# sjpollard/video-how-do-your-tokens-merge

Measured on AMD Instinct MI355X. Metric: clips/sec at r=16, VideoMAE-B 16x224x224 (forward with ToMe merge; merge indices bit-exact against the fp32-arithmetic oracle, which the reference's fp32 fixtures pin), higher is better.
Workload: dtype bf16; 1 GPU; VideoMAE-B random-init, synthetic 16x224x224 clips, r=16, bf16 (BASELINE.json configs[1]); r=16, parallelism=dp1: independent replicas, one RCCL all-reduce of [top1, top5, clips], step_launch=eager

## Files before the change

include/tome_hip.h:

```cpp
#ifndef TOME_HIP_H
#define TOME_HIP_H

#include <stddef.h>
#include <stdint.h>

#ifdef __cplusplus
extern "C" {
#endif

typedef void *tome_stream_t;

enum tome_dtype { TOME_F32 = 0, TOME_BF16 = 1, TOME_F16 = 2 };

enum tome_mode { TOME_SUM = 0, TOME_MEAN = 1, TOME_AMAX = 2, TOME_PROD = 3, TOME_AMIN = 4 };

enum tome_status {
    TOME_OK = 0,
    TOME_EINVAL = 1,
    TOME_EWORKSPACE = 2,
    TOME_ELAUNCH = 3
};

#define TOME_ABI_VERSION 11

// ... 105 lines not shown
                                  const int32_t *row_map, int drop, void *grad_in, tome_stream_t stream);

size_t tome_layernorm_backward_workspace_bytes(int64_t rows, int64_t C);
int tome_layernorm_backward(const void *gy, const void *xs, const void *gx_in, int dtype, int64_t groups,
                            int64_t group_rows, int skip_first, int64_t C, const void *weight, float eps, void *gx,
                            void *dweight, void *dbias, void *workspace, tome_stream_t stream);

size_t tome_layernorm_backward_regrouped_workspace_bytes(int64_t B, int64_t F, int64_t P, int64_t C);
int tome_layernorm_backward_regrouped(const void *gy, const void *xs, const void *gx_in, int dtype, int64_t B, int64_t F,
                                      int64_t P, int64_t C, const void *weight, float eps, void *gx, void *dweight,
                                      void *dbias, void *workspace, tome_stream_t stream);

int tome_add_layernorm_amp(const void *x, int x_dtype, const void *addend, int addend_dtype, int64_t groups,
                           int64_t group_rows, int skip_first, int64_t C, const void *weight_f32, const void *bias_f32,
                           float eps, void *x_out, void *y_out, int y_dtype, tome_stream_t stream);

size_t tome_layernorm_backward_amp_workspace_bytes(int64_t rows, int64_t C, int x_dtype);
int tome_layernorm_backward_amp(const void *gy, int gy_dtype, const void *xs, const void *gx_in, int x_dtype,
                                int64_t groups, int64_t group_rows, int skip_first, int64_t C, const void *weight_f32,
                                float eps, void *gx, void *gx16, void *dweight_f32, void *dbias_f32, void *workspace,
                                tome_stream_t stream);

size_t tome_prop_attention_backward_workspace_bytes(int64_t B, int64_t H, int64_t N, int64_t Nk);
int tome_prop_attention_backward(const void *q, const void *k, const void *v, const void *out, const void *dout,
                                 int dtype, int64_t B, int64_t H, int64_t N, int64_t Nk, int64_t D,
                                 const int64_t *q_strides, const int64_t *k_strides, const int64_t *v_strides,
                                 const int64_t *out_strides, const int64_t *dout_strides, const float *log_size,
                                 int64_t log_size_stride, int bias_skip, float scale, void *dq, void *dk, void *dv,
                                 const int64_t *dq_strides, const int64_t *dk_strides, const int64_t *dv_strides,
                                 void *workspace, size_t workspace_bytes, tome_stream_t stream);

size_t tome_prop_attention_segments_backward_workspace_bytes(int64_t B, int64_t H, int64_t N, int64_t Nk, int64_t nseg);
int tome_prop_attention_segments_backward(const void *q, const void *k, const void *v, const void *out, const void *dout,
                                          int dtype, int64_t B, int64_t H, int64_t N, int64_t Nk, int64_t D,
                                          const int64_t *q_strides, const int64_t *k_strides, const int64_t *v_strides,
                                          const int64_t *out_strides, const int64_t *dout_strides, const float *log_size,
                                          int64_t log_size_stride, float scale, int64_t nseg, const int64_t *seg_strides,
                                          const int64_t *grad_seg_strides, void *dq, void *dk, void *dv,
                                          const int64_t *dq_strides, const int64_t *dk_strides, const int64_t *dv_strides,
                                          void *workspace, size_t workspace_bytes, tome_stream_t stream);

int tome_trajectory_mix_backward(const void *q2, const void *k2, const void *val, const void *dout, int dtype, int64_t B,
                                 int64_t S, int64_t F, int64_t H, int64_t D, int64_t k_row_stride, int64_t v_row_stride,
                                 int64_t dout_batch_stride, float scale, void *dq2, void *dk2, void *dval,
                                 int64_t dk_row_stride, int64_t dv_row_stride, tome_stream_t stream);

int tome_short_attention_backward(const void *q, const void *k, const void *v, const void *dout, int dtype, int64_t B,
                                  int64_t H, int64_t N, int64_t D, const int64_t *q_strides, const int64_t *k_strides,
                                  const int64_t *v_strides, float scale, void *dq, void *dk, void *dv,
                                  const int64_t *dq_strides, const int64_t *dk_strides, const int64_t *dv_strides,
                                  tome_stream_t stream);

int tome_gelu_erf(const void *x, int dtype, int64_t elements, void *y, tome_stream_t stream);

size_t tome_gelu_erf_backward_workspace_bytes(int64_t rows, int64_t width);
int tome_gelu_erf_backward(const void *h, const void *ga, int dtype, int64_t rows, int64_t width, void *gh, void *act,
                           void *dbias, void *workspace, size_t workspace_bytes, tome_stream_t stream);

int tome_gelu_tanh(const void *x, int dtype, int64_t elements, void *y, tome_stream_t stream);
int tome_gelu_tanh_backward(const void *h, const void *ga, int dtype, int64_t rows, int64_t width, void *gh, void *act,
                            void *dbias, void *workspace, size_t workspace_bytes, tome_stream_t stream);

int tome_tubelet_rows(const void *x, int elem_bytes, int64_t B, int64_t C, int64_t T, int64_t H, int64_t W,
                      const int64_t *x_strides, int64_t kt, int64_t kh, int64_t kw, void *rows,
                      tome_stream_t stream);

int tome_row_map(int64_t n, int64_t T, int64_t r, int distill_token, const int64_t *src_idx,
                 const int64_t *dst_idx, const int64_t *unm_idx, int32_t *row_map, tome_stream_t stream);
int tome_source_init(int64_t n, int64_t T, int64_t r, int distill_token, int drop, const int32_t *row_map,
                     float *source_out, tome_stream_t stream);

size_t tome_partition_workspace_bytes(int64_t n, int64_t Na, int64_t Nb, int64_t D);
int tome_match_partition(const void *metric, int dtype, int64_t n, int64_t T, int64_t D, int64_t stride_n,
                         int64_t stride_t, int64_t k, const int64_t *a_idx, const int64_t *b_idx, int64_t Na,
                         int64_t Nb, int64_t *dst_idx, int32_t *offsets, int32_t *sources, void *workspace,
                         size_t workspace_bytes, tome_stream_t stream);
int tome_merge_partition(const void *x, int dtype, int64_t n, int64_t T, int64_t C, int64_t k, const int64_t *a_idx,
                         const int64_t *b_idx, int64_t Na, int64_t Nb, const int32_t *offsets,
                         const int32_t *sources, int mode, void *out, tome_stream_t stream);
int tome_merge_wavg_partition(const void *x, int x_dtype, const void *size, int size_dtype, int64_t n, int64_t T,
                              int64_t C, int64_t k, const int64_t *a_idx, const int64_t *b_idx, int64_t Na,
                              int64_t Nb, const int32_t *offsets, const int32_t *sources, void *x_out,
                              void *size_out, void *log_size_out, tome_stream_t stream);
int tome_unmerge_partition(const void *x, int dtype, int64_t n, int64_t T, int64_t C, int64_t k,
                           const int64_t *a_idx, const int64_t *b_idx, int64_t Na, int64_t Nb,
                           const int64_t *dst_idx, void *out, tome_stream_t stream);

#ifdef TOME_PROFILE_HOOKS
int tome_profile_enable(int on);
int tome_profile_read(float *stage_ms, int max_stages);
#endif

#ifdef __cplusplus
}
#endif
#endif
```

video-how-do-your-tokens-merge_amd/csrc/tome_kernels.hip:

```cpp
#include <hip/hip_runtime.h>
#include <stdarg.h>
#include <stdint.h>
#include <stdio.h>
#include <stdlib.h>
#include <string.h>

#include <type_traits>

#include "../../include/tome_hip.h"
#include "tome_common.h"
#include "tome_match.h"
#include "tome_match_filter.h"
#include "tome_merge.h"
#include "tome_merge_bwd.h"
#include "tome_ln_bwd.h"
#include "tome_gelu_bwd.h"
#include "tome_partition.h"
#include "tome_attn.h"
#include "tome_attn_stream.h"
#include "tome_attn_resident.h"
#include "tome_attn_bwd.h"
#include "tome_short_attn_bwd.h"
#include "tome_traj_bwd.h"
#include "tome_embed.h"

static thread_local char g_err[512] = "";

static int fail(int code, const char *fmt, ...) {
    va_list ap;
    va_start(ap, fmt);
    vsnprintf(g_err, sizeof(g_err), fmt, ap);
    va_end(ap);
    return code;
}

static int check_launch(const char *what) {
    hipError_t e = hipGetLastError();
    if (e != hipSuccess) return fail(TOME_ELAUNCH, "%s: %s", what, hipGetErrorString(e));
    return TOME_OK;
}

extern "C" int tome_abi_version(void) { return TOME_ABI_VERSION; }
extern "C" const char *tome_last_error(void) { return g_err; }

extern "C" int64_t tome_effective_r(int64_t T, int64_t r, int class_token, int distill_token) {
    int64_t prot = (class_token ? 1 : 0) + (distill_token ? 1 : 0);
    int64_t avail = T - prot;
    int64_t cap = avail >= 0 ? avail / 2 : -((-avail + 1) / 2);
    int64_t re = r < cap ? r : cap;
    return re < 0 ? 0 : re;
}

static inline size_t align_up(size_t v, size_t a) { return (v + a - 1) / a * a; }
static inline bool aligned16(const void *p) { return ((uintptr_t)p & 15) == 0; }

template <typename T> struct Dt { using type = T; };
template <int V> using Op = std::integral_constant<int, V>;

template <bool F32, typename F, typename Bad>
static int dispatch_x(int dtype, F &&f, Bad &&bad) {
    switch (dtype) {
    case TOME_F32:
        if constexpr (F32) return f(Dt<float>{});
        break;
    case TOME_BF16: return f(Dt<bf16_t>{});
    case TOME_F16: return f(Dt<f16_t>{});
    }
    return bad();
}
// ... 1260 lines not shown
        return fail(TOME_EINVAL, "tome_short_attention_backward: bad shape/pointer");
    if (D != 64 || N > SHORT_MAXN)
        return fail(TOME_EINVAL, "tome_short_attention_backward: head dim 64 and at most %d tokens per sequence",
                    SHORT_MAXN);
    if (int rc = not_16bit("tome_short_attention_backward", dtype, "tensors")) return rc;
    const int64_t *strides[6] = {q_strides, k_strides, v_strides, dq_strides, dk_strides, dv_strides};
    const void *ptrs[7] = {q, k, v, dout, dq, dk, dv};
    if (int rc = check_short_rows("tome_short_attention_backward", strides, 6, ptrs, 7)) return rc;
    for (int i = 3; i < 6; ++i)
        if ((B > 1 && strides[i][0] < H * 64) || (N > 1 && strides[i][2] < H * 64))
            return fail(TOME_EINVAL, "tome_short_attention_backward: rows of dq / dk / dv overlap");
    const int64_t units = B * H;
    const int64_t blocks = (units + 31) / 32;
    if (blocks > 0x7fffffffLL) return fail(TOME_EINVAL, "tome_short_attention_backward: too many sequences");
    const ShortBwdStrides s{q_strides[0],  q_strides[2],  k_strides[0],  k_strides[2],  v_strides[0],  v_strides[2],
                            dq_strides[0], dq_strides[2], dk_strides[0], dk_strides[2], dv_strides[0], dv_strides[2]};
    hipStream_t st = (hipStream_t)stream;
    return dispatch_x<false>(dtype, [&](auto tx) {
        using TX = typename decltype(tx)::type;
        hipLaunchKernelGGL(k_short_attention_bwd<TX>, dim3((unsigned)blocks), dim3(256), 0, st, (const TX *)q,
                           (const TX *)k, (const TX *)v, (const TX *)dout, s, units, (int)H, (int)N, scale, (TX *)dq,
                           (TX *)dk, (TX *)dv);
        return check_launch("k_short_attention_bwd");
    }, [&] { return not_16bit("tome_short_attention_backward", dtype, "tensors"); });
}

template <int FORM>
static int gelu_impl(const char *who, const void *x, int dtype, int64_t elements, void *y, tome_stream_t stream) {
    if (!x || !y || elements <= 0) return fail(TOME_EINVAL, "%s: bad shape/pointer", who);
    if (int rc = not_16bit(who, dtype, "tensors")) return rc;
    if (elements % 8 || !aligned16(x) || !aligned16(y))
        return fail(TOME_EINVAL, "%s: a multiple of 8 elements in 16-byte aligned buffers required", who);
    const int64_t chunks = elements / 8;
    const int64_t blocks = (chunks + 1023) / 1024;
    if (blocks > 0x7fffffffLL) return fail(TOME_EINVAL, "%s: too large", who);
    hipStream_t st = (hipStream_t)stream;
    return dispatch_x<false>(dtype, [&](auto tx) {
        using TX = typename decltype(tx)::type;
        if (FORM == GELU_TANH) {
            hipLaunchKernelGGL(k_gelu_tanh<TX>, dim3((unsigned)blocks), dim3(256), 0, st, (const TX *)x, (TX *)y, chunks);
            return check_launch("k_gelu_tanh");
        }
        hipLaunchKernelGGL(k_gelu_erf<TX>, dim3((unsigned)blocks), dim3(256), 0, st, (const TX *)x, (TX *)y, chunks);
        return check_launch("k_gelu_erf");
    }, [&] { return not_16bit(who, dtype, "tensors"); });
}

extern "C" int tome_gelu_erf(const void *x, int dtype, int64_t elements, void *y, tome_stream_t stream) {
    return gelu_impl<GELU_ERF>("tome_gelu_erf", x, dtype, elements, y, stream);
}

extern "C" int tome_gelu_tanh(const void *x, int dtype, int64_t elements, void *y, tome_stream_t stream) {
    return gelu_impl<GELU_TANH>("tome_gelu_tanh", x, dtype, elements, y, stream);
}

#define GELU_BWD_MAX_PARTS 512
#define GELU_BWD_MAX_WIDTH 8192
struct GeluBwdForm { int S; int U; int RP; int64_t spw; int64_t parts; };
static GeluBwdForm gelu_bwd_form(int64_t rows, int64_t width) {
    const int64_t cpr = width / 8;
    const int S = (int)((cpr + 255) / 256);
    const int U = S == 1 ? 4 : (S <= 3 ? 2 : 1);
    const int RP = S == 1 ? (int)(256 / cpr) : 1;
    const int64_t passes = (rows + RP - 1) / RP;
    const int64_t steps = (passes + U - 1) / U;
    const int64_t spw = (steps + GELU_BWD_MAX_PARTS - 1) / GELU_BWD_MAX_PARTS;
    return GeluBwdForm{S, U, RP, spw, (steps + spw - 1) / spw};
}

static bool gelu_bwd_shape_ok(int64_t rows, int64_t width) {
    return rows >= 1 && rows <= 0x7fffffffLL && width >= 8 && width % 8 == 0 && width <= GELU_BWD_MAX_WIDTH;
}

extern "C" size_t tome_gelu_erf_backward_workspace_bytes(int64_t rows, int64_t width) {
    if (!gelu_bwd_shape_ok(rows, width)) return 0;
    return align_up((size_t)gelu_bwd_form(rows, width).parts * (size_t)width * sizeof(float), 256);
}

template <int FORM>
static int gelu_backward_impl(const char *who, const void *h, const void *ga, int dtype, int64_t rows, int64_t width,
                              void *gh, void *act, void *dbias, void *workspace, size_t workspace_bytes,
                              tome_stream_t stream) {
    if (!h || !ga || !gh) return fail(TOME_EINVAL, "%s: null buffer", who);
    if (int rc = not_16bit(who, dtype, "tensors")) return rc;
    if (!gelu_bwd_shape_ok(rows, width))
        return fail(TOME_EINVAL, "%s: width %% 8 == 0, width <= 8192 and 1 .. 2^31 - 1 rows required", who);
    if (!aligned16(h) || !aligned16(ga) || !aligned16(gh) || !aligned16(act) || !aligned16(dbias) ||
        !aligned16(workspace))
        return fail(TOME_EINVAL, "%s: 16-byte aligned buffers required", who);
    if (act && (act == h || act == ga || act == gh))
        return fail(TOME_EINVAL, "%s: the activation needs a buffer of its own", who);
    if (gh == h) return fail(TOME_EINVAL, "%s: gh may lie over ga, not over h", who);
    if (dbias && (!workspace || workspace_bytes < tome_gelu_erf_backward_workspace_bytes(rows, width)))
        return fail(TOME_EWORKSPACE, "%s: the bias gradient needs a workspace of "
                                     "tome_gelu_erf_backward_workspace_bytes()", who);
    const int64_t cpr = width / 8, chunks = rows * cpr;
    hipStream_t st = (hipStream_t)stream;
    return dispatch_x<false>(dtype, [&](auto tx) {
        using TX = typename decltype(tx)::type;
        auto with_act = [&](auto launch) { return act ? launch(Op<1>{}) : launch(Op<0>{}); };
        if (!dbias) {
            const int64_t blocks = (chunks + 1023) / 1024;
            return with_act([&](auto a) {
                hipLaunchKernelGGL((k_gelu_bwd<TX, 1, false, decltype(a)::value != 0, FORM>), dim3((unsigned)blocks),
                                   dim3(256), 0, st, (const TX *)h, (const TX *)ga, chunks, 256, 1, 1, (TX *)gh, (TX *)act,
                                   (float *)nullptr);
// ... 343 lines not shown
```

video-how-do-your-tokens-merge_amd/tome/_abi.py:

```python
from __future__ import annotations

import ctypes
import os
from typing import Optional

import torch

_PKG = os.path.dirname(os.path.dirname(os.path.abspath(__file__)))
LIB_PATH = os.environ.get("TOME_HIP_LIB", os.path.join(_PKG, "lib", "libtome_hip.so"))

i64, i32, vp, sz, f32 = ctypes.c_int64, ctypes.c_int, ctypes.c_void_p, ctypes.c_size_t, ctypes.c_float
SIGNATURES = {
    "tome_abi_version": (i32, [], False),
    "tome_last_error": (ctypes.c_char_p, [], False),
    "tome_effective_r": (i64, [i64, i64, i32, i32], False),
    "tome_match_workspace_bytes": (sz, [i64, i64, i64], False),
    "tome_match": (i32, [vp, i32, i64, i64, i64, i64, i64, i64, i32, i32, vp, vp, vp, vp, vp, vp, sz, vp], False),
    "tome_match_keys": (i32, [vp, i32, i64, i64, i64, i64, i64, i64, i64, i64, i64, i64, i32, i32, vp, vp, vp, vp, vp,
                             vp, sz, vp], False),
    "tome_match_scores": (i32, [vp, i64, i64, i64, i32, i32, vp, vp, vp, vp, vp, vp, sz, vp], False),
    "tome_edge_keep": (i32, [vp, vp, i64, i64, i64, f32, vp, vp], False),
    "tome_merge_wavg": (i32, [vp, i32, vp, i32, i64, i64, i64, i64, vp, vp, vp, i32, vp, vp, vp, vp, vp], False),
    "tome_merge_wavg_ln": (i32, [vp, i32, vp, i32, i64, i64, i64, i64, vp, vp, vp, i32, vp, vp, vp, f32, vp, vp, vp, vp,
                                vp, vp, vp], False),
# ... 1 lines not shown
                                       False),
    "tome_merge_wavg_regrouped_ln": (i32, [vp, i32, vp, i32, i64, i64, i64, i64, i64, i32, vp, vp, vp, vp, vp, vp, f32,
                                          vp, i32, vp, vp, vp, vp, vp, vp, vp], False),
    "tome_add_layernorm": (i32, [vp, vp, i32, i64, i64, vp, vp, f32, vp, vp, vp], False),
    "tome_add_layernorm_skip_first": (i32, [vp, vp, i32, i64, i64, i64, vp, vp, f32, vp, vp, vp], False),
    "tome_add_layernorm_regrouped": (i32, [vp, vp, i32, i64, i64, i64, i64, vp, vp, f32, vp, vp, vp], False),
    "tome_prop_attention": (i32, [vp, vp, vp, i32, i64, i64, i64, i64, i64, vp, vp, vp, vp, i64, i32, f32, vp, vp, vp],
                                 False),
    "tome_prop_attention_segments": (i32, [vp, vp, vp, i32, i64, i64, i64, i64, i64, vp, vp, vp, vp, i64, f32, vp, vp,
                                          i64, vp, vp], False),
    "tome_trajectory_mix": (i32, [vp, vp, vp, i32, i64, i64, i64, i64, i64, i64, i64, f32, vp, i64, vp, vp], False),
    "tome_short_attention": (i32, [vp, vp, vp, i32, i64, i64, i64, i64, vp, vp, vp, f32, vp, vp], False),
    "tome_merge": (i32, [vp, i32, i64, i64, i64, i64, vp, vp, vp, i32, i32, vp, vp, vp], False),
    "tome_drop": (i32, [vp, i32, i64, i64, i64, i64, vp, i32, vp, vp], False),
    "tome_drop_regrouped": (i32, [vp, i32, i64, i64, i64, i64, i64, i32, vp, vp, vp], False),
    "tome_unmerge": (i32, [vp, i32, i64, i64, i64, i64, vp, vp, vp, vp, vp], False),
    "tome_merge_backward": (i32, [vp, i32, vp, vp, i32, i64, i64, i64, i64, vp, i32, i32, vp, vp], False),
    "tome_merge_backward_regrouped": (i32, [vp, i32, vp, vp, i32, i64, i64, i64, i64, i64, i32, vp, i32, vp, vp],
                                           False),
    "tome_row_map": (i32, [i64, i64, i64, i32, vp, vp, vp, vp, vp], False),
    "tome_source_init": (i32, [i64, i64, i64, i32, i32, vp, vp, vp], False),
    "tome_gelu_erf": (i32, [vp, i32, i64, vp, vp], False),
    "tome_tubelet_rows": (i32, [vp, i32, i64, i64, i64, i64, i64, vp, i64, i64, i64, vp, vp], False),
    "tome_partition_workspace_bytes": (sz, [i64, i64, i64, i64], False),
    "tome_match_partition": (i32, [vp, i32, i64, i64, i64, i64, i64, i64, vp, vp, i64, i64, vp, vp, vp, vp, sz, vp],
                                  False),
    "tome_merge_partition": (i32, [vp, i32, i64, i64, i64, i64, vp, vp, i64, i64, vp, vp, i32, vp, vp], False),
    "tome_merge_wavg_partition": (i32, [vp, i32, vp, i32, i64, i64, i64, i64, vp, vp, i64, i64, vp, vp, vp, vp, vp, vp],
                                       False),
    "tome_unmerge_partition": (i32, [vp, i32, i64, i64, i64, i64, vp, vp, i64, i64, vp, vp, vp], False),
    "tome_layernorm_backward_workspace_bytes": (sz, [i64, i64], True),
    "tome_layernorm_backward": (i32, [vp, vp, vp, i32, i64, i64, i32, i64, vp, f32, vp, vp, vp, vp, vp], True),
    "tome_prop_attention_backward_workspace_bytes": (sz, [i64, i64, i64, i64], True),
    "tome_prop_attention_backward": (i32, [vp, vp, vp, vp, vp, i32, i64, i64, i64, i64, i64, vp, vp, vp, vp, vp, vp,
                                          i64, i32, f32, vp, vp, vp, vp, vp, vp, vp, sz, vp], True),
    "tome_gelu_erf_backward_workspace_bytes": (sz, [i64, i64], True),
    "tome_gelu_erf_backward": (i32, [vp, vp, i32, i64, i64, vp, vp, vp, vp, sz, vp], True),
    "tome_short_attention_backward": (i32, [vp, vp, vp, vp, i32, i64, i64, i64, i64, vp, vp, vp, f32, vp, vp, vp, vp,
                                           vp, vp, vp], True),
    "tome_layernorm_backward_regrouped_workspace_bytes": (sz, [i64, i64, i64, i64], True),
    "tome_layernorm_backward_regrouped": (i32, [vp, vp, vp, i32, i64, i64, i64, i64, vp, f32, vp, vp, vp, vp, vp],
                                               True),
    "tome_prop_attention_segments_backward_workspace_bytes": (sz, [i64, i64, i64, i64, i64], True),
    "tome_prop_attention_segments_backward": (i32, [vp, vp, vp, vp, vp, i32, i64, i64, i64, i64, i64, vp, vp, vp, vp, vp,
                                                   vp, i64, f32, i64, vp, vp, vp, vp, vp, vp, vp, vp, vp, sz, vp], True),
    "tome_trajectory_mix_backward": (i32, [vp, vp, vp, vp, i32, i64, i64, i64, i64, i64, i64, i64, i64, f32, vp, vp, vp,
                                          i64, i64, vp], True),
    "tome_gelu_tanh": (i32, [vp, i32, i64, vp, vp], True),
    "tome_gelu_tanh_backward": (i32, [vp, vp, i32, i64, i64, vp, vp, vp, vp, sz, vp], True),
    "tome_add_layernorm_amp": (i32, [vp, i32, vp, i32, i64, i64, i32, i64, vp, vp, f32, vp, vp, i32, vp], True),
    "tome_layernorm_backward_amp_workspace_bytes": (sz, [i64, i64, i32], True),
    "tome_layernorm_backward_amp": (i32, [vp, i32, vp, vp, i32, i64, i64, i32, i64, vp, f32, vp, vp, vp, vp, vp, vp],
                                         True),
}
SYMBOLS = tuple(SIGNATURES)

ABI_VERSION = 11
DTYPES = {torch.float32: 0, torch.bfloat16: 1, torch.float16: 2}
MODES = {"sum": 0, "mean": 1, "amax": 2, "max": 2, "prod": 3, "amin": 4, "min": 4}

_lib = None


class TomeHipError(RuntimeError):
    pass


def lib() -> ctypes.CDLL:
    global _lib
    if _lib is not None:
        return _lib
    _lib = bind(LIB_PATH)
    return _lib


def bind(path: str) -> ctypes.CDLL:
    if not os.path.exists(path):
        raise TomeHipError(
            f"HIP extension not found at {path}: the MI355X merge path has no fallback. "
            "Build it with `python video-how-do-your-tokens-merge_amd/csrc/build.py` (needs hipcc).")
    L = ctypes.CDLL(path)
    for name, (restype, argtypes, later) in SIGNATURES.items():
        if later and not _exports(L, name):
            continue
        fn = getattr(L, name)
        fn.restype, fn.argtypes = restype, argtypes
    if L.tome_abi_version() != ABI_VERSION:
        raise TomeHipError(f"{os.path.basename(path)} ABI {L.tome_abi_version()} != expected {ABI_VERSION}")
    return L


def _exports(L, name: str) -> bool:
    try:
        getattr(L, name)
    except AttributeError:
        return False
    return True


def require_symbol(L, name: str):
    if not _exports(L, name):
        raise TomeHipError(f"{name} is missing from the loaded library: it reports ABI {ABI_VERSION} but was built before "
                           "this entry was added; rebuild it with `python video-how-do-your-tokens-merge_amd/csrc/build.py`")
    return getattr(L, name)


# ... 824 lines not shown
        rc = entry(q2.data_ptr(), k2.data_ptr(), val.data_ptr(), dout.data_ptr(), dtype_code(q2, "q2"), B, S, F, heads, 64,
                   k2.stride(2), val.stride(2), dout.stride(0) if B > 1 else 0, float(scale), dq2.data_ptr(), _ptr(dk2),
                   _ptr(dval), 0 if dk2 is None else dk2.stride(2), 0 if dval is None else dval.stride(2),
                   _stream(q2.device))
    _check(rc, "tome_trajectory_mix_backward")
    return dq2, dk2, dval


def drop_regrouped(plan: MatchPlan, x_full: torch.Tensor, frames: int, has_cls: bool = True) -> torch.Tensor:
    x_full, B, C, cls, F, P = _prep_regrouped("drop_regrouped", plan, x_full, frames, has_cls)
    out = torch.empty((B, cls + (P - plan.r) * F, C), dtype=x_full.dtype, device=x_full.device)
    with _on_device(x_full.device):
        rc = lib().tome_drop_regrouped(x_full.data_ptr(), dtype_code(x_full, "x"), B, F, P, C, plan.r, cls,
                                       plan.unm_idx.data_ptr(), out.data_ptr(), _stream(x_full.device))
    _check(rc, "tome_drop_regrouped")
    return out


def unmerge(plan: MatchPlan, x: torch.Tensor) -> torch.Tensor:
    x = _prep_x(plan, x, "unmerge(x)", plan.T - plan.r)
    n, _, C = x.shape
    out = torch.empty((n, plan.T, C), dtype=x.dtype, device=x.device)
    with _on_device(x.device):
        rc = lib().tome_unmerge(x.data_ptr(), dtype_code(x, "x"), n, plan.T, C, plan.r, plan.src_idx.data_ptr(),
                                plan.dst_idx.data_ptr(), plan.unm_idx.data_ptr(), out.data_ptr(), _stream(x.device))
    _check(rc, "tome_unmerge")
    return out


def gelu_ok(x: torch.Tensor) -> bool:
    return (x.is_cuda and x.dtype in (torch.bfloat16, torch.float16) and x.is_contiguous() and x.numel() % 8 == 0
            and x.numel() > 0 and x.data_ptr() % 16 == 0 and not (torch.is_grad_enabled() and needs_grad(x)))


def _gelu(name: str, x: torch.Tensor, inplace: bool) -> torch.Tensor:
    if not gelu_ok(x):
        raise TomeHipError(f"{name}: contiguous 16-bit device tensor with a multiple of 8 elements required")
    entry = require_symbol(lib(), "tome_" + name)
    y = x if inplace else torch.empty_like(x)
    with _on_device(x.device):
        rc = entry(x.data_ptr(), dtype_code(x, "x"), x.numel(), y.data_ptr(), _stream(x.device))
    _check(rc, "tome_" + name)
    return y


def gelu_erf(x: torch.Tensor, inplace: bool = False) -> torch.Tensor:
    return _gelu("gelu_erf", x, inplace)


def gelu_tanh(x: torch.Tensor, inplace: bool = False) -> torch.Tensor:
    return _gelu("gelu_tanh", x, inplace)


GELU_BWD_MAX_WIDTH = 8192


def mlp_trainable(y: torch.Tensor, fc1, fc2, act) -> bool:
    from ._mlp import _stock_module
    if not (_stock_module(fc1, torch.nn.Linear) and _stock_module(fc2, torch.nn.Linear)
            and _stock_module(act, torch.nn.GELU) and getattr(act, "approximate", "none") == "none"):
        return False
    return mlp_tensors_trainable(y, fc1, fc2)


def mlp_tensors_trainable(y: torch.Tensor, fc1, fc2) -> bool:
    C, Hd = fc1.in_features, fc1.out_features
    params = [fc1.weight, fc2.weight] + [b for b in (fc1.bias, fc2.bias) if b is not None]
    return (y.is_cuda and y.dtype in (torch.bfloat16, torch.float16) and y.dim() >= 2 and y.shape[-1] == C
            and y.numel() > 0 and fc2.in_features == Hd and Hd % 8 == 0 and Hd <= GELU_BWD_MAX_WIDTH
            and (C * y.element_size()) % 16 == 0 and (fc2.out_features * y.element_size()) % 16 == 0
            and all(p.dtype == y.dtype and p.device == y.device for p in params))


def _gelu_backward(name: str, h: torch.Tensor, ga: torch.Tensor, want_act: bool, want_bias: bool, inplace: bool):
    require_device(h, f"{name}(h)")
    if h.dtype not in (torch.bfloat16, torch.float16):
        raise TomeHipError(f"{name}: 16-bit tensors only, got {h.dtype}")
    Hd = h.shape[-1] if h.dim() >= 2 else 0
    if Hd == 0 or Hd % 8 or Hd > GELU_BWD_MAX_WIDTH or h.numel() == 0:
        raise TomeHipError(f"{name}: h must be [..., Hd] with Hd % 8 == 0 and Hd <= {GELU_BWD_MAX_WIDTH}, "
                           f"got {tuple(h.shape)}")
    if ga.shape != h.shape or ga.dtype != h.dtype or ga.device != h.device:
        raise TomeHipError(f"{name}: ga must have h's shape, dtype and device")
    if not h.is_contiguous() or not ga.is_contiguous():
        raise TomeHipError(f"{name}: contiguous tensors required")
    h, ga = h.detach(), ga.detach()
    rows = h.numel() // Hd
    L = lib()
    entry = require_symbol(L, "tome_" + name)
    gh = ga if inplace else torch.empty_like(ga)
    act = torch.empty_like(h) if want_act else None
    dbias = torch.empty(Hd, dtype=h.dtype, device=h.device) if want_bias else None
    with _on_device(h.device):
        stream = _stream(h.device)
        ws = _sized_workspace(L, "tome_gelu_erf_backward_workspace_bytes", (rows, Hd), h.device, stream,
                              name) if want_bias else None
        rc = entry(h.data_ptr(), ga.data_ptr(), dtype_code(h, "h"), rows, Hd, gh.data_ptr(), _ptr(act), _ptr(dbias),
                   _ptr(ws), 0 if ws is None else ws.numel(), stream)
    _check(rc, "tome_" + name)
    return gh, act, dbias


def gelu_erf_backward(h: torch.Tensor, ga: torch.Tensor, *, want_act: bool, want_bias: bool, inplace: bool = True):
    return _gelu_backward("gelu_erf_backward", h, ga, want_act, want_bias, inplace)


# ... 328 lines not shown
```

video-how-do-your-tokens-merge_amd/tome/patch/_common.py:

```python
from __future__ import annotations

import os
import threading
from typing import Callable, Dict, Tuple

import torch

from .. import _abi, _attn, _ln, _mlp, _overlap
from .._mlp import _plain_mlp, _stock_module
from ..merge import (bipartite_soft_matching, bipartite_soft_matching_drop, bipartite_soft_matching_hybrid,
                     drop_regrouped, merge_source, merge_wavg, merge_wavg_regrouped)
from ..utils import parse_r

_SUBCLASSES: Dict[Tuple[type, str], type] = {}
_FUSE_LN = os.environ.get("TOME_FUSE_LN", "1") != "0"
_FUSE_ADD = os.environ.get("TOME_FUSE_ADD", "1") != "0"
_FUSE_NEXT = os.environ.get("TOME_FUSE_NEXT", "1") != "0"
_ATTN_KERNEL = os.environ.get("TOME_ATTN_KERNEL", "1") != "0"
_GELU_KERNEL = os.environ.get("TOME_GELU_KERNEL", "1") != "0"
_FUSE_FC2 = os.environ.get("TOME_FUSE_FC2", "1") != "0"
_SKIP_FIRST = os.environ.get("TOME_SKIP_FIRST", "1") != "0"


def swizzle(module: torch.nn.Module, tag: str, methods: dict) -> None:
    base = module.__class__
    if getattr(base, "_tome_tag", None) == tag:
        return
    key = (base, tag)
    sub = _SUBCLASSES.get(key)
    if sub is None:
        sub = type(tag, (base,), dict(methods, _tome_tag=tag))
        _SUBCLASSES[key] = sub
    module.__class__ = sub


def has_tag(module, tag: str) -> bool:
    return getattr(module.__class__, "_tome_tag", None) == tag


def new_tome_info(trace_source, prop_attn, mode, head_aggregation, threshold, verbose, class_token) -> dict:
    return {
        "r": 0,
        "size": None,
        "source": None,
        "trace_source": trace_source,
        "prop_attn": prop_attn,
        "verbose": verbose,
        "class_token": class_token,
        "distill_token": False,
        "mode": mode,
        "head_aggregation": head_aggregation,
        "threshold": threshold,
    }


_in_flight = {}
_issue_locks: Dict[int, "threading.RLock"] = {}
_issue_locks_guard = threading.Lock()
_warned_two_streams = False


def _current_stream(device):
    cur = torch.cuda.current_stream(device)
    return cur.cuda_stream, cur


def _record_event(stream):
    ev = torch.cuda.Event()
    ev.record(stream)
    return ev


def _guarded(device) -> bool:
# ... 7 lines not shown
            lock = _issue_locks[device.index] = threading.RLock()
        return lock


def _guard_one_forward_in_flight(device) -> None:
    global _warned_two_streams
    sid, cur = _current_stream(device)
    last = _in_flight.get(device.index)
    if last is None or last[0] == sid or last[1].query():
        return
    msg = ("a forward issued on another HIP stream of this process is still in flight: the library GEMMs of two "
           "concurrent forwards never finish on this platform")
    if os.environ.get("TOME_ONE_FORWARD", "order") == "raise":
        raise RuntimeError(msg + ".  Run one forward at a time per process (one process per GPU).")
    cur.wait_event(last[1])
    if not _warned_two_streams:
        _warned_two_streams = True
        import warnings
        warnings.warn(msg + "; this forward has been ordered behind it (no overlap between the two streams).",
                      RuntimeWarning, stacklevel=3)


def _note_forward_issued(device) -> None:
    sid, cur = _current_stream(device)
    _in_flight[device.index] = (sid, _record_event(cur))


class one_forward_at_a_time:

    def __init__(self, device):
        self.device = device
        self.on = device is not None and _guarded(device)

    def __enter__(self):
        if self.on:
            self.lock = _issue_lock(self.device)
            self.lock.acquire()
            try:
                _guard_one_forward_in_flight(self.device)
            except BaseException:
                self.lock.release()
                raise
        return self

    def __exit__(self, *exc):
        if self.on:
            try:
                _note_forward_issued(self.device)
            finally:
                self.lock.release()
        return False


def wrap_model_forward(model_wrapper: torch.nn.Module, blocks_of: Callable) -> None:
    base = model_wrapper.__class__
    if getattr(base, "_tome_tag", None) == "ToMeVisionTransformer":
        return

    def forward(self, *args, **kwdargs):
        param = next(self.parameters(), None)
        with one_forward_at_a_time(None if param is None else param.device):
            self._tome_info["r"] = parse_r(len(blocks_of(self)), self.r)
            self._tome_info["size"] = None
            self._tome_info["source"] = None
            self._tome_info.pop("_prenorm", None)
            self._tome_info.pop("_folded", None)
            try:
                return super(sub, self).forward(*args, **kwdargs)
            finally:
                if param is not None:
                    _overlap.join(param.device)

    sub = type("ToMeVisionTransformer", (base,), {"forward": forward, "_tome_tag": "ToMeVisionTransformer"})
    model_wrapper.__class__ = sub


keys_ready = _overlap.keys_ready
match_beside = _overlap.match_beside


def attention_qkv(qkv, size, scale: float, dropout_p: float = 0.0, bias_skip: bool = False):
    return attention(qkv[0], qkv[1], qkv[2], size, scale, dropout_p, bias_skip, qkv)


def attention(q, k, v, size, scale: float, dropout_p: float = 0.0, bias_skip: bool = False, qkv=None):
    out = _attn.attention(q, k, v, size, scale, dropout_p, bias_skip, qkv) if _ATTN_KERNEL else None
    if out is not None:
        return out
    B, H, N, hd = q.shape
    bias = None
    if size is not None:
        log = _abi.log_of_size(size)[:, None, None, :, 0].to(q.dtype)
        if bias_skip:
            bias = torch.zeros(B, 1, N, N, dtype=q.dtype, device=q.device)
            bias[:, :, 1:, 1:] = log
        else:
            bias = log
    out = torch.nn.functional.scaled_dot_product_attention(q, k, v, attn_mask=bias, dropout_p=dropout_p, scale=scale)
    return out.transpose(1, 2).reshape(B, N, H * hd)


def _mlp_steps(mlp, y):
    return mlp.fc2(_mlp.hidden(mlp, y, _GELU_KERNEL)) if _plain_mlp(mlp) else mlp(y)


def run_mlp(mlp, y):
    out = _mlp.mlp(mlp, y) if _GELU_KERNEL else None
    return _mlp_steps(mlp, y) if out is None else out


def foldable(linear, eval_mode: bool = True):
    if (_FUSE_FC2 and _FUSE_NEXT and eval_mode and _stock_module(linear, torch.nn.Linear) and linear.bias is not None
            and not (torch.is_grad_enabled() and _abi.needs_grad(linear.weight, linear.bias))):
        return linear
    return None


def mlp_residual(block, mlp, x, y, info, scale=None, drop_path=None):
    folded = info.get("_folded")
    waiting = folded is not None and folded[0] is x
    out = _mlp.mlp(mlp, y) if _GELU_KERNEL and not waiting else None
    if out is None:
        if _plain_mlp(mlp) and scale is None and (drop_path is None or not block.training):
            return finish_linear(block, x, _mlp.hidden(mlp, y, _GELU_KERNEL), mlp.fc2, info)
        if waiting:
            raise RuntimeError("the residual stream carries a folded bias, but the block's MLP is not the one it was folded for")
        out = _mlp_steps(mlp, y)
    if scale is not None:
        out = scale * out
    return finish_block(block, x, out if drop_path is None else drop_path(out), info)


def pick_reduction(mode: str, merge_fn, drop_fn, hybrid_fn):
    if mode in ("merge", "random_merge"):
        return merge_fn
    if mode in ("drop", "random_drop"):
        return drop_fn
    if mode in ("hybrid",):
        return hybrid_fn
    raise ValueError(f"unknown ToMe mode {mode!r}")


def reduce_merge(metric, x, info, r):
    merge, _ = bipartite_soft_matching(metric, r, info["class_token"], info["distill_token"], info["mode"])
    if info["trace_source"]:
        info["source"] = merge_source(merge, x, info["source"])
    before = x.size(1)
    x, info["size"] = merge_wavg(merge, x, info["size"], log_size=info["prop_attn"])
    if info["verbose"]:
        print(f"Merged {before} to {x.size(1)} tokens")
    return x


def link_next_norms(blocks, norm_attr: str, tag: str = "ToMeBlock", skip_first: bool = False) -> None:
    blocks = list(blocks)
    for cur, nxt in zip(blocks, blocks[1:]):
        target = getattr(nxt, norm_attr, None) if has_tag(nxt, tag) and nxt is not cur else None
        object.__setattr__(cur, "_tome_next_norm", target)
        object.__setattr__(cur, "_tome_next_skip_first", bool(skip_first) and _SKIP_FIRST)
    if blocks:
        object.__setattr__(blocks[-1], "_tome_next_norm", None)


def first_norm(block, x, info, norm, skip_first: bool = False):
    pre = info.pop("_prenorm", None)
    if pre is not None and pre[0] is x and pre[2] is norm:
        if bool(pre[3]) == bool(skip_first):
            return pre[1]
        if skip_first:
            return pre[1][:, 1:, :]
    out = _ln.add_layernorm(x, None, norm, skip_first) if _FUSE_NEXT else None
    if out is None:
        return norm(x)[:, 1:, :] if skip_first else norm(x)
    _, y, skipped = out
    return y[:, 1:, :] if (skip_first and not skipped) else y


def _hand_over(block, x, addend, info):
    nxt = getattr(block, "_tome_next_norm", None)
    out = None if nxt is None else _ln.add_layernorm(x, addend, nxt, getattr(block, "_tome_next_skip_first", False))
    if out is None:
        return None
    x, h, skipped = out
# ... 215 lines not shown
```

video-how-do-your-tokens-merge_amd/tome/patch/videomae.py:

```python
from __future__ import annotations

import copy

import torch
import torch.nn.functional as F

from . import _common as C
from ..merge import HeadMeanKeys


def _block_forward(self, x):
    info = self._tome_info
    attn_size = info["size"] if info["prop_attn"] else None
    attn, metric = self.attn(C.first_norm(self, x, info, self.norm1), attn_size, info["head_aggregation"])
    if self.gamma_1 is not None:
        attn = self.gamma_1 * attn
    fold = C.foldable(self.mlp.fc2, not self.training) if (self.gamma_2 is None and C._plain_mlp(self.mlp)) else None
    x, y = C.merge_then_norm(metric, x, info, self.norm2, self.reduction_function, videomae_merge,
                             residual=self.drop_path(attn), fold=fold)
    return C.mlp_residual(self, self.mlp, x, y, info, scale=self.gamma_2, drop_path=self.drop_path)


def _duplicate_block_forward(self, x):
    info = self._tome_info
    attn_size = info["size"] if info["prop_attn"] else None
    _, metric = self.attn(self.norm1(x), attn_size, info["head_aggregation"])
    return self.reduction_function(metric, x, info)


def _attention_forward(self, x, size: torch.Tensor = None, head_aggregation: str = "mean"):
    B, N, _ = x.shape
    bias = None
    if self.q_bias is not None:
        bias = torch.cat((self.q_bias, torch.zeros_like(self.v_bias, requires_grad=False), self.v_bias))
    qkv = F.linear(x, self.qkv.weight, bias).reshape(B, N, 3, self.num_heads, -1).permute(2, 0, 3, 1, 4)
    q, k, v = qkv[0], qkv[1], qkv[2]
    drop_p = self.attn_drop.p if self.training else 0.0
    info = getattr(self, "_tome_info", None)
    ready = C.keys_ready(k, info) if head_aggregation == "mean" else None
    out = C.attention_qkv(qkv, size, self.scale, drop_p)
    if head_aggregation == "mean":
        metric = HeadMeanKeys(k)
        C.match_beside(metric, ready, info)
    elif head_aggregation == "concat":
        metric = k.transpose(1, 2).reshape(B, N, -1)
    else:
        raise ValueError(f"head_aggregation {head_aggregation!r}")
    return self.proj_drop(self.proj(out)), metric


def videomae_merge(metric, x, _tome_info):
    r = _tome_info["r"].pop(0)
    return C.reduce_merge(metric, x, _tome_info, r) if r > 0 else x


def videomae_drop(metric, x, _tome_info):
    r = _tome_info["r"].pop(0)
    return C.reduce_drop(metric, x, _tome_info, r) if r > 0 else x


def videomae_hybrid(metric, x, _tome_info):
    r = _tome_info["r"].pop(0)
    return C.reduce_hybrid(metric, x, _tome_info, r) if r > 0 else x


def _is_block(m) -> bool:
    return all(hasattr(m, a) for a in ("attn", "mlp", "norm1", "norm2", "gamma_1"))


def _is_attention(m) -> bool:
    return all(hasattr(m, a) for a in ("qkv", "proj", "num_heads", "q_bias"))


def apply_duplicate_patch(model, layer_to_duplicate, quantity):
    for i in range(layer_to_duplicate, layer_to_duplicate + quantity - 1):
        model.model.blocks.insert(index=i, module=copy.deepcopy(model.model.blocks[i]))
        C.swizzle(model.model.blocks[i], "ToMeDuplicateBlock", {"forward": _duplicate_block_forward})


def apply_patch(model_wrapper, trace_source: bool = False, prop_attn: bool = False, mode: str = "merge",
                head_aggregation: str = "mean", threshold: float = 0.0, verbose: bool = False):
    model = model_wrapper.model
    C.wrap_model_forward(model_wrapper, lambda w: w.model.blocks)
    model_wrapper.r = 0
    model_wrapper._tome_info = C.new_tome_info(trace_source, prop_attn, mode, head_aggregation, threshold, verbose,
                                               class_token=False)
    reduction_function = C.pick_reduction(mode, videomae_merge, videomae_drop, videomae_hybrid)
    for module in model.modules():
        if C.has_tag(module, "ToMeDuplicateBlock"):
            module._tome_info = model_wrapper._tome_info
            module.reduction_function = reduction_function
        elif _is_block(module):
            C.swizzle(module, "ToMeBlock", {"forward": _block_forward})
            module._tome_info = model_wrapper._tome_info
            module.reduction_function = reduction_function
        elif _is_attention(module):
            C.swizzle(module, "ToMeAttention", {"forward": _attention_forward})
            module._tome_info = model_wrapper._tome_info
    C.link_next_norms(model.blocks, "norm1")
```

Measured before the change: 2575 clips/s.

## Pool the last block's MLP output before fc2 using linearity of mean pooling

For the final transformer block in eval mode, the model ends with an identity norm followed by mean pooling and fc_norm. The MLP's fc2 and the residual add are both linear, so the change averages GELU(fc1(y)) and x over tokens with a new HIP token_mean kernel, then runs fc2 once per clip on the pooled vector instead of per token. This drops the per-token fc2 GEMM and the residual write in the last block, and returns a single pooled token so the host's mean step becomes trivial. In exchange it relies on a number of module-type and hook checks, and its rounding differs from the original per-token bf16 path because the sum is accumulated in fp32.

```diff
diff --git a/include/tome_hip.h b/include/tome_hip.h
--- a/include/tome_hip.h
+++ b/include/tome_hip.h
@@ -181,6 +181,9 @@
                                   tome_stream_t stream);
 
 int tome_gelu_erf(const void *x, int dtype, int64_t elements, void *y, tome_stream_t stream);
+
+int tome_token_mean(const void *x, int dtype, int64_t groups, int64_t tokens, int64_t width, int act, float *out,
+                    tome_stream_t stream);
 
 size_t tome_gelu_erf_backward_workspace_bytes(int64_t rows, int64_t width);
 int tome_gelu_erf_backward(const void *h, const void *ga, int dtype, int64_t rows, int64_t width, void *gh, void *act,
diff --git a/video-how-do-your-tokens-merge_amd/csrc/tome_kernels.hip b/video-how-do-your-tokens-merge_amd/csrc/tome_kernels.hip
--- a/video-how-do-your-tokens-merge_amd/csrc/tome_kernels.hip
+++ b/video-how-do-your-tokens-merge_amd/csrc/tome_kernels.hip
@@ -15,6 +15,7 @@
 #include "tome_merge_bwd.h"
 #include "tome_ln_bwd.h"
 #include "tome_gelu_bwd.h"
+#include "tome_token_mean.h"
 #include "tome_partition.h"
 #include "tome_attn.h"
 #include "tome_attn_stream.h"
@@ -1381,6 +1382,32 @@
 
 extern "C" int tome_gelu_tanh(const void *x, int dtype, int64_t elements, void *y, tome_stream_t stream) {
     return gelu_impl<GELU_TANH>("tome_gelu_tanh", x, dtype, elements, y, stream);
+}
+
+extern "C" int tome_token_mean(const void *x, int dtype, int64_t groups, int64_t tokens, int64_t width, int act,
+                               float *out, tome_stream_t stream) {
+    if (!x || !out) return fail(TOME_EINVAL, "tome_token_mean: null pointer");
+    if (int rc = not_16bit("tome_token_mean", dtype, "tensors")) return rc;
+    if (act != TOKEN_MEAN_NONE && act != TOKEN_MEAN_GELU_ERF)
+        return fail(TOME_EINVAL, "tome_token_mean: act must be 0 (none) or 1 (exact-erf GELU), got %d", act);
+    if (groups < 1 || tokens < 1 || width < 8 || width % 8)
+        return fail(TOME_EINVAL, "tome_token_mean: groups >= 1, tokens >= 1 and width %% 8 == 0 required");
+    if (!aligned16(x) || ((uintptr_t)out & 3))
+        return fail(TOME_EINVAL, "tome_token_mean: x must be 16-byte aligned, out 4-byte aligned");
+    const int64_t slabs = (width + TOKEN_MEAN_SLAB - 1) / TOKEN_MEAN_SLAB;
+    if (width > 0x7fffffffLL - TOKEN_MEAN_SLAB || tokens > 0x7fffffffLL || groups > 0x7fffffffLL / slabs
+        || groups > INT64_MAX / tokens / width)
+        return fail(TOME_EINVAL, "tome_token_mean: too large");
+    hipStream_t st = (hipStream_t)stream;
+    return dispatch_x<false>(dtype, [&](auto tx) {
+        using TX = typename decltype(tx)::type;
+        auto launch = [&](auto a) {
+            hipLaunchKernelGGL((k_token_mean<TX, decltype(a)::value>), dim3((unsigned)(groups * slabs)), dim3(256), 0, st,
+                               (const TX *)x, tokens, (int)width, (int)slabs, out);
+            return check_launch("k_token_mean");
+        };
+        return act == TOKEN_MEAN_GELU_ERF ? launch(Op<TOKEN_MEAN_GELU_ERF>{}) : launch(Op<TOKEN_MEAN_NONE>{});
+    }, [&] { return not_16bit("tome_token_mean", dtype, "tensors"); });
 }
 
 #define GELU_BWD_MAX_PARTS 512
diff --git a/video-how-do-your-tokens-merge_amd/csrc/tome_token_mean.h b/video-how-do-your-tokens-merge_amd/csrc/tome_token_mean.h
--- /dev/null
+++ b/video-how-do-your-tokens-merge_amd/csrc/tome_token_mean.h
@@ -0,0 +1,61 @@
+#pragma once
+
+enum { TOKEN_MEAN_NONE = 0, TOKEN_MEAN_GELU_ERF = 1 };
+#define TOKEN_MEAN_SLAB 512
+
+template <typename TX, int ACT>
+__global__ __launch_bounds__(256) void k_token_mean(const TX *__restrict__ x, int64_t tokens, int width, int slabs,
+                                                    float *__restrict__ out) {
+    constexpr int VEC = 8;
+    constexpr int WAVES = 4;
+    constexpr int U = 8;
+    static_assert(sizeof(TX) == 2, "16-bit tokens");
+    __shared__ float part[WAVES - 1][VEC * WAVE];
+    const int lane = threadIdx.x & (WAVE - 1), wave = threadIdx.x >> 6;
+    const int64_t g = blockIdx.x / slabs;
+    const int slab = (int)(blockIdx.x - g * slabs);
+    const int c0 = slab * TOKEN_MEAN_SLAB + lane * VEC;
+    const bool live = c0 < width;
+    float sum[VEC];
+#pragma unroll
+    for (int e = 0; e < VEC; ++e) sum[e] = 0.0f;
+    if (live) {
+        const TX *base = x + g * tokens * width + c0;
+        for (int64_t t0 = wave; t0 < tokens; t0 += WAVES * U) {
+            uint4 raw[U];
+#pragma unroll
+            for (int u = 0; u < U; ++u) {
+                const int64_t t = t0 + u * WAVES;
+                if (t < tokens) raw[u] = ld16(base + t * width);
+            }
+#pragma unroll
+            for (int u = 0; u < U; ++u) {
+                if (t0 + u * WAVES >= tokens) continue;
+                Pack<TX, VEC> pk;
+                __builtin_memcpy(&pk, &raw[u], 16);
+#pragma unroll
+                for (int e = 0; e < VEC; ++e) {
+                    float v = to_f32(pk.e[e]);
+                    if (ACT == TOKEN_MEAN_GELU_ERF)
+                        v = to_f32(from_f32<TX>(fp32_value(gelu_erf_value(v, gelu_erf_one_plus(v)))));
+                    sum[e] += v;
+                }
+            }
+        }
+    }
+    if (wave > 0) {
+#pragma unroll
+        for (int e = 0; e < VEC; ++e) part[wave - 1][e * WAVE + lane] = sum[e];
+    }
+    __syncthreads();
+    if (wave == 0 && live) {
+        const float n = (float)tokens;
+        float *o = out + g * width + c0;
+#pragma unroll
+        for (int e = 0; e < VEC; ++e) {
+#pragma unroll
+            for (int w = 0; w < WAVES - 1; ++w) sum[e] += part[w][e * WAVE + lane];
+            o[e] = sum[e] / n;
+        }
+    }
+}
diff --git a/video-how-do-your-tokens-merge_amd/tome/_abi.py b/video-how-do-your-tokens-merge_amd/tome/_abi.py
--- a/video-how-do-your-tokens-merge_amd/tome/_abi.py
+++ b/video-how-do-your-tokens-merge_amd/tome/_abi.py
@@ -77,6 +77,7 @@
     "tome_layernorm_backward_amp_workspace_bytes": (sz, [i64, i64, i32], True),
     "tome_layernorm_backward_amp": (i32, [vp, i32, vp, vp, i32, i64, i64, i32, i64, vp, f32, vp, vp, vp, vp, vp, vp],
                                          True),
+    "tome_token_mean": (i32, [vp, i32, i64, i64, i64, i32, vp, vp], True),
 }
 SYMBOLS = tuple(SIGNATURES)
 
@@ -1007,6 +1008,24 @@
     return _gelu("gelu_tanh", x, inplace)
 
 
+def token_mean_ok(x: torch.Tensor) -> bool:
+    return (x.is_cuda and x.dim() == 3 and x.dtype in _HALF and x.is_contiguous() and x.numel() > 0
+            and x.shape[-1] % 8 == 0 and x.data_ptr() % 16 == 0 and not (torch.is_grad_enabled() and needs_grad(x)))
+
+
+def token_mean(x: torch.Tensor, gelu: bool = False) -> torch.Tensor:
+    if not token_mean_ok(x):
+        raise TomeHipError("token_mean: contiguous 16-bit [groups, tokens, width] device tensor with width % 8 == 0 "
+                           f"required, got {tuple(x.shape)} {x.dtype} on {x.device}")
+    groups, tokens, width = x.shape
+    entry = require_symbol(lib(), "tome_token_mean")
+    out = torch.empty((groups, width), dtype=torch.float32, device=x.device)
+    with _on_device(x.device):
+        rc = entry(x.data_ptr(), DTYPES[x.dtype], groups, tokens, width, int(bool(gelu)), out.data_ptr(), _stream(x.device))
+    _check(rc, "tome_token_mean")
+    return out
+
+
 GELU_BWD_MAX_WIDTH = 8192
 
 
diff --git a/video-how-do-your-tokens-merge_amd/tome/patch/_common.py b/video-how-do-your-tokens-merge_amd/tome/patch/_common.py
--- a/video-how-do-your-tokens-merge_amd/tome/patch/_common.py
+++ b/video-how-do-your-tokens-merge_amd/tome/patch/_common.py
@@ -19,6 +19,7 @@
 _ATTN_KERNEL = os.environ.get("TOME_ATTN_KERNEL", "1") != "0"
 _GELU_KERNEL = os.environ.get("TOME_GELU_KERNEL", "1") != "0"
 _FUSE_FC2 = os.environ.get("TOME_FUSE_FC2", "1") != "0"
+_POOL_TAIL = os.environ.get("TOME_POOL_TAIL", "1") != "0"
 _SKIP_FIRST = os.environ.get("TOME_SKIP_FIRST", "1") != "0"
 
 
@@ -132,7 +133,7 @@
         return False
 
 
-def wrap_model_forward(model_wrapper: torch.nn.Module, blocks_of: Callable) -> None:
+def wrap_model_forward(model_wrapper: torch.nn.Module, blocks_of: Callable, pool_tail: Callable = None) -> None:
     base = model_wrapper.__class__
     if getattr(base, "_tome_tag", None) == "ToMeVisionTransformer":
         return
@@ -145,9 +146,13 @@
             self._tome_info["source"] = None
             self._tome_info.pop("_prenorm", None)
             self._tome_info.pop("_folded", None)
+            armed = pool_tail(self) if (pool_tail is not None and _POOL_TAIL) else None
+            if armed is not None:
+                self._tome_info["_pool_tail"] = armed
             try:
                 return super(sub, self).forward(*args, **kwdargs)
             finally:
+                self._tome_info.pop("_pool_tail", None)
                 if param is not None:
                     _overlap.join(param.device)
 
@@ -209,6 +214,44 @@
     if scale is not None:
         out = scale * out
     return finish_block(block, x, out if drop_path is None else drop_path(out), info)
+
+
+def _unhooked(*modules) -> bool:
+    return not any(m._forward_hooks or m._forward_pre_hooks for m in modules)
+
+
+def pool_tail_modules_ok(vit, block) -> bool:
+    from torch.nn.modules import module as _m
+    if _m._global_forward_hooks or _m._global_forward_pre_hooks:
+        return False
+    norm, fc_norm = getattr(vit, "norm", None), getattr(vit, "fc_norm", None)
+    if not (type(norm) is torch.nn.Identity and isinstance(fc_norm, torch.nn.LayerNorm) and not vit.training
+            and not block.training and has_tag(block, "ToMeBlock") and getattr(block, "gamma_2", 0) is None
+            and type(getattr(block, "drop_path", None)) is torch.nn.Identity
+            and _unhooked(vit, norm, block, block.drop_path) and _plain_mlp(block.mlp)):
+        return False
+    fc1, fc2, norm2 = block.mlp.fc1, block.mlp.fc2, getattr(block, "norm2", None)
+    dtype = fc2.weight.dtype
+    return (fc2.bias is not None and dtype in _abi._HALF and fc1.weight.dtype == dtype
+            and isinstance(norm2, torch.nn.LayerNorm) and norm2.elementwise_affine and norm2.weight.dtype == dtype
+            and fc1.in_features % 8 == 0 and fc1.out_features % 8 == 0 and fc2.out_features == fc1.in_features)
+
+
+def pool_tail_armed(block, x, info) -> bool:
+    if info.get("_pool_tail") is not block:
+        return False
+    info.pop("_pool_tail")
+    return (x.is_cuda and x.dim() == 3 and x.dtype == block.mlp.fc2.weight.dtype and not torch.is_grad_enabled()
+            and not torch.is_autocast_enabled("cuda"))
+
+
+def pooled_tail(mlp, x, y):
+    h = mlp.fc1(y)
+    abar = _abi.token_mean(h if h.is_contiguous() else h.contiguous(), gelu=True)
+    xbar = _abi.token_mean(x if x.is_contiguous() else x.contiguous())
+    fc2 = mlp.fc2
+    pooled = torch.addmm(xbar + fc2.bias.float(), abar, fc2.weight.float().t())
+    return pooled.to(x.dtype)[:, None, :]
 
 
 def pick_reduction(mode: str, merge_fn, drop_fn, hybrid_fn):
diff --git a/video-how-do-your-tokens-merge_amd/tome/patch/videomae.py b/video-how-do-your-tokens-merge_amd/tome/patch/videomae.py
--- a/video-how-do-your-tokens-merge_amd/tome/patch/videomae.py
+++ b/video-how-do-your-tokens-merge_amd/tome/patch/videomae.py
@@ -1,6 +1,7 @@
 from __future__ import annotations
 
 import copy
+import sys
 
 import torch
 import torch.nn.functional as F
@@ -15,9 +16,13 @@
     attn, metric = self.attn(C.first_norm(self, x, info, self.norm1), attn_size, info["head_aggregation"])
     if self.gamma_1 is not None:
         attn = self.gamma_1 * attn
-    fold = C.foldable(self.mlp.fc2, not self.training) if (self.gamma_2 is None and C._plain_mlp(self.mlp)) else None
+    pooled = C.pool_tail_armed(self, x, info)
+    fold = (C.foldable(self.mlp.fc2, not self.training)
+            if (not pooled and self.gamma_2 is None and C._plain_mlp(self.mlp)) else None)
     x, y = C.merge_then_norm(metric, x, info, self.norm2, self.reduction_function, videomae_merge,
                              residual=self.drop_path(attn), fold=fold)
+    if pooled:
+        return C.pooled_tail(self.mlp, x, y)
     return C.mlp_residual(self, self.mlp, x, y, info, scale=self.gamma_2, drop_path=self.drop_path)
 
 
@@ -64,6 +69,22 @@
     return C.reduce_hybrid(metric, x, _tome_info, r) if r > 0 else x
 
 
+def pooled_tail_block(wrapper):
+    if torch.is_grad_enabled():
+        return None
+    host = sys.modules.get("hosts.videomae")
+    vit = getattr(wrapper, "model", None)
+    if (host is None or type(vit) is not host.VisionTransformer or type(wrapper).__bases__ != (host.VideoMAE,)
+            or "forward" in vit.__dict__ or "forward_features" in vit.__dict__ or "forward" in wrapper.__dict__
+            or len(vit.blocks) == 0):
+        return None
+    block = vit.blocks[-1]
+    if (getattr(block, "_tome_info", None) is not wrapper._tome_info or "forward" in block.__dict__
+            or any(b is block for b in vit.blocks[:-1])):
+        return None
+    return block if C.pool_tail_modules_ok(vit, block) else None
+
+
 def _is_block(m) -> bool:
     return all(hasattr(m, a) for a in ("attn", "mlp", "norm1", "norm2", "gamma_1"))
 
@@ -81,7 +102,7 @@
 def apply_patch(model_wrapper, trace_source: bool = False, prop_attn: bool = False, mode: str = "merge",
                 head_aggregation: str = "mean", threshold: float = 0.0, verbose: bool = False):
     model = model_wrapper.model
-    C.wrap_model_forward(model_wrapper, lambda w: w.model.blocks)
+    C.wrap_model_forward(model_wrapper, lambda w: w.model.blocks, pool_tail=pooled_tail_block)
     model_wrapper.r = 0
     model_wrapper._tome_info = C.new_tome_info(trace_source, prop_attn, mode, head_aggregation, threshold, verbose,
                                                class_token=False)
```

Measured after the change: 2606 clips/s, median of 6. +1.2%, better.
